# kakaoenterprise/JORLDY

Measured on AMD Instinct MI355X. Metric: env_steps_per_s (PPO CartPole sync, W=8 workers/GPU, T=128), higher is better.
Workload: dtype f32

## Files before the change

jorldy_amd/csrc/jh_collect.hip:

```cpp
#include <chrono>

#include "jh_common.h"

struct jh_persist;
int jh_persist_create(jh_pponet* n, jh_persist** out);
void jh_persist_destroy(jh_persist* p);
int jh_persist_begin(jh_persist* p, int W, int T, hipStream_t st, int split = 0);
unsigned jh_persist_publish(jh_persist* p, int W, const float* h_obs);
unsigned jh_persist_seq(const jh_persist* p);
void jh_persist_publish_rows(jh_persist* p, int r0, int r1, const float* h_obs, unsigned tag);
int jh_persist_collect_range(jh_persist* p, int r0, int n_rows, unsigned tag, float* h_heads);
int jh_persist_collect(jh_persist* p, int W, unsigned tag, float* h_heads);
int jh_persist_collect_rows(jh_persist* p, const int* rows, int n_rows, unsigned tag, float* h_heads);
void jh_persist_abort(jh_persist* p);
bool jh_persist_gave_up(const jh_persist* p);
void jh_persist_dump_debug(jh_persist* p, int T);

namespace {
struct Level {
  void* env = nullptr;
  int S = 0;
  std::vector<float> next, obs, rw;
  std::vector<uint8_t> dn;
  std::vector<int64_t> act;
  void init(int rows, int S_) {
    S = S_;
    next.resize((size_t)S * rows); obs.resize((size_t)S * rows); rw.resize(rows); dn.resize(rows); act.resize(rows);
    for (int i = 0; i < rows; ++i) act[i] = i & 1;
  }
};
inline int fork_step(const jh_env_vtbl& vt, Level& dst, const void* src, int n_src) {
  for (int i = 0; i < n_src; ++i) { vt.copy_row(dst.env, 2 * i, src, i); vt.copy_row(dst.env, 2 * i + 1, src, i); }
  int rc = vt.step(dst.env, 0, 2 * n_src, dst.act.data(), dst.next.data(), dst.rw.data(), dst.dn.data());
  if (rc) return rc;
  return vt.obs(dst.env, 0, 2 * n_src, dst.obs.data());
}
inline void copy_level_row(const jh_env_vtbl& vt, Level& d, int di, const Level& s_, int si) {
  vt.copy_row(d.env, di, s_.env, si);
  const size_t S = (size_t)d.S;
  memcpy(&d.next[S * (size_t)di], &s_.next[S * (size_t)si], sizeof(float) * S);
  memcpy(&d.obs[S * (size_t)di], &s_.obs[S * (size_t)si], sizeof(float) * S);
  d.rw[di] = s_.rw[si];
  d.dn[di] = s_.dn[si];
}
}

struct jh_collector {
  jh_ctx* ctx = nullptr;
  jh_pponet* net = nullptr;
  jh_env_vtbl vt{};
// ... 1 lines not shown
  jh_store* store = nullptr;
  int W = 0, S = 0, A = 0;
  int no = 0;
  bool cont = false;
  int col_state = 0, col_action = 1, col_reward = 2, col_next = 3, col_done = 4;
  std::vector<float> obs, next_obs, reward, heads, act_f;
  std::vector<int64_t> act_i;
  std::vector<uint8_t> done;
  bool dbg = false, dbg_persist = false;
  double dbg_publish = 0.0, dbg_wait = 0.0;
  long dbg_n = 0;
  jh_persist* persist = nullptr;
  int mode = 1;
  int lookahead = 1;
  bool split = false;
  Level lv[4];
  void *spec = nullptr, *spec2 = nullptr, *spec3 = nullptr;
  float *cap_h0 = nullptr, *cap_h1 = nullptr, *cap_v = nullptr, *cap_nv = nullptr;
  int64_t cap_rows = 0;
  const void* ride_src[2] = {nullptr, nullptr};
  void* ride_dst[2] = {nullptr, nullptr};
  int64_t ride_bytes[2] = {0, 0};
  void* run = nullptr;
  unsigned *gate_h = nullptr, *gate_d = nullptr, gate_seq = 0;
  int prelaunched_T = 0;
  double t_act = 0, t_env = 0, t_total = 0;
  double t_first = 0, t_extra = 0, t_commit = 0;
  int64_t runs = 0;
  int64_t steps = 0;
};
// ... 28 lines not shown
  c->dbg = getenv("JH_COLLECT_DEBUG") != nullptr;
  c->dbg_persist = getenv("JH_PERSIST_DEBUG") != nullptr;
  if (const char* e = getenv("JH_COLLECT_PERSISTENT")) c->mode = atoi(e);
  if (c->mode == 1 && W <= 32 && W * S <= 512) {
    if (jh_persist_create(net, &c->persist) != JH_OK) c->persist = nullptr;
  }
  const bool forkable = vt->fork_alloc && vt->fork_free && vt->copy_row;
  if (c->persist && forkable && !cont && A == 2 && 3 * W <= 32 && 3 * W * S <= 128) {
    const char* e = getenv("JH_COLLECT_LOOKAHEAD");
    c->lookahead = e ? (atoi(e) >= 2 ? 2 : 1) : 2;
    if (c->lookahead == 2) {
      c->spec = vt->fork_alloc(env, 2 * W); c->spec2 = vt->fork_alloc(env, 4 * W); c->spec3 = vt->fork_alloc(env, 8 * W);
      if (!c->spec || !c->spec2 || !c->spec3) c->lookahead = 1;
    }
  }
  {
    const char* e = getenv("JH_COLLECT_SPLIT");
    c->split = c->persist && c->lookahead != 2 && W == 32 && (vt->obs == cart_obs || vt->obs == ctl_obs) && !(e && atoi(e) == 0);
  }
  c->obs.resize((size_t)S * W);
  c->next_obs.resize((size_t)S * W);
  c->act_i.resize(W);
  c->act_f.resize((size_t)A * W);
  c->reward.resize(W);
  c->done.resize(W);
  c->heads.resize((size_t)c->no * W);
  run_state_alloc(c);
  *out = c;
  return JH_OK;
}

static int cart_obs(void* e, int32_t r0, int32_t r1, float* o) { jh_cartpole_obs_rows((const jh_cartpole*)e, r0, r1, o); return JH_OK; }
static int cart_step(void* e, int32_t r0, int32_t r1, const void* a, float* nx, float* rw, uint8_t* dn) {
// ... 72 lines not shown
  JH_ARG(c != nullptr && slot >= 0 && slot < 2 && bytes >= 0 && (bytes == 0 || (d_src_mapped && d_dst)));
  c->ride_src[slot] = d_src_mapped; c->ride_dst[slot] = d_dst; c->ride_bytes[slot] = bytes;
  return JH_OK;
}

static int collector_steps(const jh_collector* c, int T) {
  const int extra = (c->cap_v && c->cap_rows == (int64_t)c->W * T) ? 1 : 0;
  return (c->lookahead == 2 ? (T + 1) / 2 : T) + extra;
}
static int collector_rows(const jh_collector* c) { return c->lookahead == 2 ? 3 * c->W : c->W; }

JH_EXPORT int jh_collector_prelaunch(jh_collector* c, int32_t T, jh_stream stream) {
  JH_ARG(c != nullptr && T > 0);
  if (!c->persist || c->prelaunched_T) return JH_OK;
  const int steps = collector_steps(c, T);
  int rc = jh_persist_begin(c->persist, collector_rows(c), steps, jh_s(stream), c->split);
  if (rc == JH_OK) c->prelaunched_T = steps;
  return rc;
}

struct RunState {
  bool active = false, cap = false, persistent = false, early = false;
  int T = 0, steps = 0;
  int64_t n = 0;
  float *st = nullptr, *ns = nullptr, *rw = nullptr;
  uint8_t* dn = nullptr;
  int64_t* ac_i = nullptr;
  float* ac_f = nullptr;
  jh_pinned_slab* cap_slab = nullptr;
  float *ch0 = nullptr, *ch1 = nullptr, *cv = nullptr, *cnv = nullptr;
  int stall_t = -1, stall_h = -1;
// ... 63 lines not shown
    if (rc) { (void)jh_store_stage_commit(c->store, st); return rc; }
    r.ch0 = (float*)r.cap_slab->host;
    r.ch1 = c->cont ? r.ch0 + (size_t)r.n * A : nullptr;
    r.cv = r.ch0 + (size_t)r.n * A * (c->cont ? 2 : 1);
    r.cnv = r.cv + r.n;
  }
  r.persistent = c->persist != nullptr;
  if (r.persistent) {
    const int pre = c->prelaunched_T;
    c->prelaunched_T = 0;
    if (pre != r.steps || jh_persist_gave_up(c->persist)) {
      if (pre && !jh_persist_gave_up(c->persist)) {
        jh_persist_abort(c->persist);
        (void)hipStreamSynchronize(st);
      }
      rc = jh_persist_begin(c->persist, collector_rows(c), r.steps, st, c->split);
      if (rc) r.persistent = false;
    }
  }
  r.active = true;
  return JH_OK;
}

using Clock = std::chrono::steady_clock;
static double secs(Clock::time_point a, Clock::time_point b) { return std::chrono::duration<double>(b - a).count(); }

static void count_act(jh_collector* c, const RunState& r, int t, double dt) {
  c->t_act += dt;
  if (t == r.T) c->t_extra += dt;
  else if (t == 0) c->t_first += dt;
}
// ... 102 lines not shown
    c->steps += 1;
  }
  *t_done = steps;
  if (c->dbg_persist && (c->runs % 16) == 15) jh_persist_dump_debug(c->persist, T);
  if (c->dbg_n > 0 && (c->runs % 4) == 3) {
    fprintf(stderr, "[jh_collect] one timestep per exchange, per step: publish %.2f us, wait + read of the heads %.2f us (sampling + bookkeeping + env step: the rest of act / env)\n",
            c->dbg_publish / c->dbg_n * 1e6, c->dbg_wait / c->dbg_n * 1e6);
    c->dbg_publish = c->dbg_wait = 0.0;
    c->dbg_n = 0;
  }
  return JH_OK;
}

static int run_loop_split(jh_collector* c, int training, hipStream_t st, int* t_done) {
  RunState& r = run_state(c);
  const int W = c->W, T = r.T, steps = T + (r.cap ? 1 : 0), HR = 16;
  const unsigned base = jh_persist_seq(c->persist);
  bool dead = false;
  int rc = c->vt.obs(c->env, 0, W, c->obs.data());
  if (rc) return env_failed(c, rc);
  for (int h = 0; h < 2; ++h) jh_persist_publish_rows(c->persist, h * HR, (h + 1) * HR, c->obs.data(), base + 1);
  for (int t = 0; t < steps; ++t) {
    const bool extra = t == T;
    for (int h = 0; h < 2; ++h) {
      const int r0 = h * HR, r1 = r0 + HR;
      const auto t0 = Clock::now();
      if (t == r.stall_t && h == r.stall_h) {
        while (secs(t0, Clock::now()) < 0.35) {}
      }
      rc = jh_persist_collect_range(c->persist, r0, HR, base + (unsigned)t + 1, c->heads.data() + (size_t)r0 * c->no);
      if (rc) {
        rc = kernel_gave_up(c, r, t, st, t_done);
        if (rc || h == 0) return rc;
        const uint64_t ctr = c->net->act_ctr;
        rc = act_launch(c, r0, HR, 0, st);
        if (rc) return rc;
        c->net->act_ctr = ctr;
        dead = true;
      }
      for (int w = r0; w < r1; ++w) {
        const float* z = c->heads.data() + (size_t)w * c->no;
        if (!extra) sample_row(c, z, w, training);
        capture_row(c, r, w, t, z);
      }
      if (h == 1 && !extra) c->net->act_ctr += 1;
      const auto t1 = Clock::now();
      count_act(c, r, t, secs(t0, t1));
      if (extra) continue;
      rc = step_rows(c, r, r0, r1, t);
      if (rc) return env_failed(c, rc);
      if (t + 1 < steps && !dead) {
        rc = c->vt.obs(c->env, r0, r1, c->obs.data());
        if (rc) return env_failed(c, rc);
        jh_persist_publish_rows(c->persist, r0, r1, c->obs.data(), base + (unsigned)t + 2);
      }
      c->t_env += secs(t1, Clock::now());
    }
    if (!extra) c->steps += 1;
    if (dead) {
      *t_done = t + 1;
      return JH_OK;
    }
  }
  *t_done = steps;
  return JH_OK;
}

static int run_loop_lookahead(jh_collector* c, int training, hipStream_t st, int* t_done) {
  RunState& r = run_state(c);
  const int W = c->W, S = c->S, T = r.T, steps = T + (r.cap ? 1 : 0), no = c->no;
  void* e = c->env;
  const jh_env_vtbl& vt = c->vt;
  Level &L1 = c->lv[0], &L2 = c->lv[1], &L3 = c->lv[2], &tmp = c->lv[3];
  L1.env = c->spec; L2.env = c->spec2; L3.env = c->spec3;
  L1.init(2 * W, S); L2.init(4 * W, S); L3.init(8 * W, S);
  std::vector<float> pub((size_t)3 * W * S), pub_next((size_t)3 * W * S), hz((size_t)W * no), hz2((size_t)W * no);
  std::vector<int> pick(W);
  std::vector<int64_t> a0(W), a1(W);
  int t = 0;
  const bool dbg = c->dbg;
  double d_fork = 0, d_wait = 0, d_sample = 0, d_publish = 0, d_book = 0;
  int n_ex = 0;
  int rc = fork_step(vt, L1, e, W);
  if (!rc) rc = vt.obs(e, 0, W, pub.data());
  if (rc) return env_failed(c, rc);
  memcpy(pub.data() + (size_t)W * S, L1.obs.data(), sizeof(float) * (size_t)2 * W * S);
  auto t0 = Clock::now();
  unsigned tag = jh_persist_publish(c->persist, 3 * W, pub.data());
  while (t < steps) {
    const bool extra = t == T;
    const bool two = !extra && t + 1 < T;
    const int t_next = t + (two ? 2 : 1);
    const auto q0 = dbg ? Clock::now() : Clock::time_point();
    if (!extra) {
      rc = fork_step(vt, L2, L1.env, 2 * W);
      if (!rc && two && t_next < steps) rc = fork_step(vt, L3, L2.env, 4 * W);
      if (rc) return env_failed(c, rc);
    }
    const auto q1 = dbg ? Clock::now() : q0;
    rc = jh_persist_collect_rows(c->persist, nullptr, W, tag, hz.data());
    const auto q2 = dbg ? Clock::now() : q0;
    if (rc) return kernel_gave_up(c, r, t, st, t_done);
    if (!extra) {
      for (int w = 0; w < W; ++w) {
        a0[w] = jh_sample_discrete(c->net, hz.data() + (size_t)w * no, w, training);
        pick[w] = W + 2 * w + (int)a0[w];
      }
      c->net->act_ctr += 1;
      if (two) {
        rc = jh_persist_collect_rows(c->persist, pick.data(), W, tag, hz2.data());
        if (rc) return rc;
// ... 52 lines not shown
    if (!two)
      for (int i = 0; i < 2 * W; ++i) copy_level_row(vt, L1, i, tmp, i);
    c->steps += two ? 2 : 1;
    const auto t2 = Clock::now();
    if (dbg) d_book += secs(q3, t2);
    c->t_env += secs(t1, t2);
    t = t_next;
    tag = tag_next;
    t0 = t0_next;
    pub.swap(pub_next);
  }
  *t_done = t;
  if (dbg && n_ex > 0 && (c->runs % 16) == 15)
    fprintf(stderr, "[jh_collect] host us per exchange (%d exchanges): fork %.2f  wait %.2f  sample %.2f  publish %.2f  book %.2f\n", n_ex, d_fork / n_ex * 1e6,
            d_wait / n_ex * 1e6, d_sample / n_ex * 1e6, d_publish / n_ex * 1e6, d_book / n_ex * 1e6);
  if (c->dbg_persist && (c->runs % 16) == 15) jh_persist_dump_debug(c->persist, collector_steps(c, T));
  return JH_OK;
}

static int run_loop_per_launch(jh_collector* c, int training, hipStream_t st, int t_begin) {
  RunState& r = run_state(c);
  if (r.early) return jh_fail(JH_ERR_STATE, "jh_collector_begin needs the persistent acting kernel (W <= 32, W * S <= 512, JH_COLLECT_PERSISTENT != 0)");
  const int W = c->W, T = r.T, steps = T + (r.cap ? 1 : 0);
  for (int t = t_begin; t < steps; ++t) {
    const bool extra = t == T;
    int rc = c->vt.obs(c->env, 0, W, c->obs.data());
    if (rc) return rc;
    const auto t0 = Clock::now();
    rc = act_launch(c, 0, W, training, st);
    if (rc) return rc;
// ... 2 lines not shown
    const auto t1 = Clock::now();
    count_act(c, r, t, secs(t0, t1));
    if (extra) break;
    rc = step_rows(c, r, 0, W, t);
    if (rc) return rc;
    c->t_env += secs(t1, Clock::now());
    c->steps += 1;
  }
  return JH_OK;
}

static int run_loop(jh_collector* c, int training, hipStream_t st) {
  RunState& r = run_state(c);
  int t = 0;
  if (r.persistent) {
    const int rc = c->lookahead == 2 ? run_loop_lookahead(c, training, st, &t)
                   : c->split        ? run_loop_split(c, training, st, &t)
                                     : run_loop_exchange(c, training, st, &t);
    if (rc) return rc;
  }
  return t < r.T + (r.cap ? 1 : 0) ? run_loop_per_launch(c, training, st, t) : JH_OK;
}

JH_EXPORT int jh_collector_run(jh_collector* c, int32_t T, int32_t training, jh_stream stream) {
  JH_ARG(c != nullptr && T > 0);
  if (run_state(c).active) return jh_fail(JH_ERR_STATE, "jh_collector_run inside a jh_collector_begin / jh_collector_loop pair");
  int rc = run_prepare(c, T, jh_s(stream));
  if (rc) return rc;
  rc = run_loop(c, training, jh_s(stream));
  const auto tc = std::chrono::steady_clock::now();
  rc = run_commit(c, run_state(c), rc, nullptr, 0, jh_s(stream));
// ... 75 lines not shown
```

jorldy_amd/csrc/jh_common.h:

```cpp
#pragma once
#include <hip/hip_runtime.h>
#include <math.h>
#include <stdint.h>
#include <stdio.h>
#include <string.h>

#include <deque>
#include <mutex>
#include <string>
#include <vector>

#include "../../include/jorldy_hip.h"

#define JH_EXPORT extern "C" __attribute__((visibility("default")))

std::string& jh_err_slot();
int jh_fail(int code, const char* fmt, ...);

#define JH_HIP(expr)                                                                          \
  do {                                                                                        \
    hipError_t _e = (expr);                                                                   \
    if (_e != hipSuccess)                                                                     \
      return jh_fail(JH_ERR_HIP, "%s:%d %s -> %s", __FILE__, __LINE__, #expr, hipGetErrorString(_e)); \
  } while (0)
// ... 143 lines not shown
  float* xg = nullptr;
  float* tg_ws = nullptr;
  size_t tg_ws_floats = 0;
  unsigned* tg_cnt = nullptr;
  int tg_cnt_slots = 0;
};

static inline uint64_t jh_mix64(uint64_t x) {
  x += 0x9E3779B97F4A7C15ull;
  x = (x ^ (x >> 30)) * 0xBF58476D1CE4E5B9ull;
  x = (x ^ (x >> 27)) * 0x94D049BB133111EBull;
  return x ^ (x >> 31);
}
static inline double jh_u01_of(uint64_t key) { return (double)(jh_mix64(key) >> 11) * (1.0 / 9007199254740992.0); }

static inline int64_t jh_sample_discrete(const jh_pponet* n, const float* z, int wq, int training) {
  const int A = n->A;
  int act = 0;
  float mx = z[0];
  for (int k = 1; k < A; ++k)
    if (z[k] > mx) { mx = z[k]; act = k; }
  if (!training) return act;
  float e[40], se = 0.f;
  for (int k = 0; k < A; ++k) { e[k] = expf(z[k] - mx); se += e[k]; }
  const float u = (float)jh_u01_of(n->act_seed * 0x100000001B3ull + n->act_ctr * 0x9E3779B97F4A7C15ull + (uint64_t)wq) * se;
  float c = 0.f;
  act = A - 1;
  for (int k = 0; k < A; ++k) {
    c += e[k];
    if (u < c) { act = k; break; }
  }
  return act;
}

static inline void jh_sample_continuous(const jh_pponet* n, const float* z, int wq, int training, float* action) {
  const int A = n->A;
  for (int k = 0; k < A; ++k) {
    const float mu = fminf(fmaxf(z[k], -5.f), 5.f);
    float v = mu;
    if (training) {
      const float sd = expf(tanhf(z[A + k]));
      const uint64_t key = n->act_seed * 0x100000001B3ull + n->act_ctr * 0x9E3779B97F4A7C15ull + (uint64_t)wq * 64u + (uint64_t)k;
      const double u1 = 1.0 - jh_u01_of(key * 2 + 1), u2 = jh_u01_of(key * 2 + 2);
      v = mu + sd * (float)(sqrt(-2.0 * log(u1)) * cos(6.283185307179586 * u2));
    }
    action[k] = tanhf(v);
  }
}
// ... 75 lines not shown
```

jorldy_amd/csrc/jh_persist.hip:

```cpp
#if defined(__x86_64__)
#include <emmintrin.h>
#endif

#include "jh_common.h"

typedef float f32x4 __attribute__((ext_vector_type(4)));

struct PersistArgs {
  int W, S, H, n_out, T, G;
  const float *W1, *b1, *W2, *b2;
  const float* wh[12];
  const float* hbias[12];
  const unsigned long long* obs_gran;
  float4* part;
  int rows_ld;
  unsigned* abort_flag;
  unsigned seq0;
  long max_polls;
  unsigned long long* dbg;
  int period;
  unsigned long long* mbox;
  float4* dpart;
  int split;
};

__device__ __forceinline__ void persist_poll_issue(const void* gsrc, unsigned lds_off) {
  unsigned keep;
  asm volatile("s_mov_b32 %0, m0\n\ts_mov_b32 m0, %2\n\ts_nop 0\n\tglobal_load_lds_dwordx4 %1, off sc0 sc1\n\ts_mov_b32 m0, %0"
               : "=&s"(keep) : "v"(gsrc), "s"(lds_off) : "memory");
}

template <int SP, int NCH, int D, int PI>
__global__ void __launch_bounds__(256, 1) jh_act_persist_kernel(PersistArgs p) {
  constexpr bool W1LDS = SP > 8;
  constexpr int NJ = 2 * PI;
  __shared__ __attribute__((aligned(16))) unsigned long long s_ring[D][128 * PI];
  __shared__ __attribute__((aligned(16))) float s_w1[W1LDS ? 64 * NCH * SP : 4];
  __shared__ __attribute__((aligned(16))) float s_x[2][16][SP];
// ... 29 lines not shown
      const int k = i / SP, q = i - k * SP;
      s_w1[i] = q < S ? p.W1[(size_t)k * S + q] : 0.f;
    }
  }
  for (int i = threadIdx.x; i < 12 * 16; i += 256) {
    const int o = i >> 4, c = i & 15;
    s_wh[o][c] = o < p.n_out ? p.wh[o][n0 + c] : 0.f;
  }
  if (threadIdx.x < 16) s_b2[threadIdx.x] = p.b2[n0 + threadIdx.x];
  if (threadIdx.x < 12) s_hb[threadIdx.x] = threadIdx.x < p.n_out ? *p.hbias[threadIdx.x] : 0.f;
  for (int i = threadIdx.x; i < 2 * 16 * SP; i += 256) (&s_x[0][0][0])[i] = 0.f;
  for (int i = threadIdx.x; i < D * 128 * PI; i += 256) (&s_ring[0][0])[i] = 0ull;
  __syncthreads();

  const int g0 = p.split ? rt * 16 * S : 0;
  const int n_gran = p.split ? (p.W - 16 * rt < 16 ? p.W - 16 * rt : 16) * S : p.W * S;
  const int n16 = (n_gran + 1) >> 1;
  const char* my_src = reinterpret_cast<const char*>(p.obs_gran + g0) + 16 * (lane < n16 ? lane : 0);
  const bool poller = !p.mbox || (p.split ? tile == 0 : blockIdx.x == 0);
  unsigned long long next_issue = 0;
  int slot = 0;
  const unsigned ring_lane = (unsigned)(uintptr_t)&s_ring[0][0] + 8u * (unsigned)lane;
  __builtin_amdgcn_s_waitcnt(0x0F70);
  if (wid == 0 && poller) {
#pragma unroll
    for (int d = 0; d < D; ++d) {
#pragma unroll
      for (int q = 0; q < PI; ++q)
        if (64 * q + lane < n16) persist_poll_issue(my_src + 1024 * q, __builtin_amdgcn_readfirstlane((unsigned)(uintptr_t)&s_ring[d][0]) + 1024u * q);
    }
    next_issue = wall_clock64();
// ... 127 lines not shown
      __builtin_amdgcn_fence(__ATOMIC_RELEASE, "workgroup");
      f32x4 ph = (f32x4){0.f, 0.f, 0.f, 0.f};
#pragma unroll
      for (int c = 0; c < 4; ++c) {
        const float av = s_h2[r][4 * c + kq];
        const float bv = r < 12 ? s_wh[r][4 * c + kq] : 0.f;
        ph = __builtin_amdgcn_mfma_f32_16x16x4f32(av, bv, ph, 0, 0, 0);
      }
      if (r < 12) {
#pragma unroll
        for (int i = 0; i < 4; ++i) s_out[kq * 4 + i][r] = ph[i] + (tile == 0 ? s_hb[r] : 0.f);
      }
      __builtin_amdgcn_wave_barrier();
      __builtin_amdgcn_fence(__ATOMIC_RELEASE, "workgroup");
      const int g = lane >> 4, row = lane & 15;
      if (g < p.G && 16 * rt + row < p.W) {
        const f32x4 gq = (f32x4){s_out[row][3 * g], s_out[row][3 * g + 1], s_out[row][3 * g + 2], __uint_as_float(tag)};
        if (p.dpart) {
          float4* dst = p.dpart + ((size_t)(rt * p.G + g) * 16 + row) * tiles_n + tile;
          asm volatile("global_store_dwordx4 %0, %1, off sc1\n\ts_nop 1" ::"v"(dst), "v"(gq) : "memory");
        } else {
          float4* dst = p.part + ((size_t)tile * p.G + g) * p.rows_ld + 16 * rt + row;
          asm volatile("global_store_dwordx4 %0, %1, off sc0 sc1\n\ts_nop 1" ::"v"(dst), "v"(gq) : "memory");
        }
      }
    }
    if (p.dpart && tile == 0) {
      const int g = lane >> 4, row = lane & 15;
      const bool mine = g < p.G && 16 * rt + row < p.W;
      const int per = tiles_n / 4;
      bool ok = true;
      if (mine) {
        const float4* src = p.dpart + ((size_t)(rt * p.G + g) * 16 + row) * tiles_n + wid * per;
        f32x4 q[8];
        long spin = 0;
        for (;;) {
          const float4* a1 = per > 4 ? src + 4 : src;
          asm volatile("global_load_dwordx4 %0, %8, off sc1\n\tglobal_load_dwordx4 %1, %9, off sc1\n\tglobal_load_dwordx4 %2, %10, off sc1\n\t"
                       "global_load_dwordx4 %3, %11, off sc1\n\tglobal_load_dwordx4 %4, %12, off sc1\n\tglobal_load_dwordx4 %5, %12, off offset:16 sc1\n\t"
                       "global_load_dwordx4 %6, %12, off offset:32 sc1\n\tglobal_load_dwordx4 %7, %12, off offset:48 sc1\n\ts_waitcnt vmcnt(0)"
                       : "=&v"(q[0]), "=&v"(q[1]), "=&v"(q[2]), "=&v"(q[3]), "=&v"(q[4]), "=&v"(q[5]), "=&v"(q[6]), "=&v"(q[7])
                       : "v"(src), "v"(src + (per > 1 ? 1 : 0)), "v"(src + (per > 2 ? 2 : 0)), "v"(src + (per > 2 ? 3 : 0)), "v"(a1)
                       : "memory");
          bool all = true, newer = false;
// ... 21 lines not shown
          good = good && __float_as_uint(v[3]) == tag;
          z0 += v[0]; z1 += v[1]; z2 += v[2];
        }
        if (good) {
          const f32x4 gq = (f32x4){z0, z1, z2, __uint_as_float(tag)};
          float4* dst = p.part + (size_t)g * p.rows_ld + 16 * rt + row;
          asm volatile("global_store_dwordx4 %0, %1, off sc0 sc1\n\ts_nop 1" ::"v"(dst), "v"(gq) : "memory");
        }
      }
    }
    if (p.dbg && blockIdx.x == 0 && threadIdx.x == 0) { p.dbg[(t - 1) * 8 + 4] = wall_clock64(); p.dbg[(t - 1) * 8 + 5] = __builtin_readcyclecounter(); }
  }
  asm volatile("s_waitcnt vmcnt(0)" ::: "memory");
}

constexpr int kPersistMaxGranules = 512;
struct jh_persist {
  jh_pponet* net = nullptr;
  unsigned long long* gran_h = nullptr;
  unsigned long long* gran_d = nullptr;
  float4 *part_h = nullptr, *part_d = nullptr;
  unsigned *flag_h = nullptr, *flag_d = nullptr;
  unsigned seq = 0;
  int tiles = 0, n_out = 0, G = 0;
  int rows_ld = 16;
  unsigned long long *dbg_h = nullptr, *dbg_d = nullptr;
  unsigned long long* mbox = nullptr;
  float4* dpart = nullptr;
  bool reduced = false;
  int rows_published = 0;
// ... 40 lines not shown
  (void)hipHostFree(p->part_h);
  (void)hipHostFree(p->flag_h);
  (void)hipFree(p->mbox);
  (void)hipFree(p->dpart);
  if (p->dbg_d) (void)hipFree(p->dbg_d);
  free(p->dbg_h);
  delete p;
}

template <int SP, int NCH>
static void persist_launch(int depth, int pi, int grid, hipStream_t st, const PersistArgs& a) {
  if (pi == 2) JH_LAUNCH_NAMED("jh_act_persist_kernel", (jh_act_persist_kernel<SP, NCH, 4, 2>), dim3(grid), dim3(256), 0, st, a);
  else if (pi == 3) JH_LAUNCH_NAMED("jh_act_persist_kernel", (jh_act_persist_kernel<SP, NCH, 4, 3>), dim3(grid), dim3(256), 0, st, a);
  else if (pi == 4) JH_LAUNCH_NAMED("jh_act_persist_kernel", (jh_act_persist_kernel<SP, NCH, 4, 4>), dim3(grid), dim3(256), 0, st, a);
  else if (depth >= 4) JH_LAUNCH_NAMED("jh_act_persist_kernel", (jh_act_persist_kernel<SP, NCH, 4, 1>), dim3(grid), dim3(256), 0, st, a);
  else if (depth >= 2) JH_LAUNCH_NAMED("jh_act_persist_kernel", (jh_act_persist_kernel<SP, NCH, 2, 1>), dim3(grid), dim3(256), 0, st, a);
  else JH_LAUNCH_NAMED("jh_act_persist_kernel", (jh_act_persist_kernel<SP, NCH, 1, 1>), dim3(grid), dim3(256), 0, st, a);
}

int jh_persist_begin(jh_persist* p, int W, int T, hipStream_t st, int split) {
  jh_pponet* n = p->net;
  JH_ARG(W > 0 && W <= 32 && W * n->S <= kPersistMaxGranules && T > 0 && (!split || W == 32));
  const int win = split ? 16 * n->S : W * n->S;
  const int pi = ((win + 1) / 2 + 63) / 64;
  PersistArgs a{};
  a.W = W; a.S = n->S; a.H = n->H; a.T = T; a.G = p->G;
  a.W1 = n->params + n->o_w1; a.b1 = n->params + n->o_b1; a.W2 = n->params + n->o_w2; a.b2 = n->params + n->o_b2;
  int o = 0;
  for (int k = 0; k < n->A; ++k, ++o) { a.wh[o] = n->params + n->o_wh0 + (int64_t)k * n->H; a.hbias[o] = n->params + n->o_bh0 + k; }
  if (n->cont)
    for (int k = 0; k < n->A; ++k, ++o) { a.wh[o] = n->params + n->o_wh1 + (int64_t)k * n->H; a.hbias[o] = n->params + n->o_bh1 + k; }
  a.wh[o] = n->params + n->o_wv; a.hbias[o] = n->params + n->o_bv; ++o;
  a.n_out = o;
  a.obs_gran = p->gran_d; a.part = p->part_d; a.abort_flag = p->flag_d;
  a.seq0 = p->seq;
  a.dbg = p->dbg_d;
  static const int depth = getenv("JH_PERSIST_DEPTH") ? atoi(getenv("JH_PERSIST_DEPTH")) : 4;
  static const int period = getenv("JH_PERSIST_PERIOD") ? atoi(getenv("JH_PERSIST_PERIOD")) : 10;
  a.period = depth > 1 ? period : 0;
  static const int relay = getenv("JH_PERSIST_RELAY") ? atoi(getenv("JH_PERSIST_RELAY")) : 1;
  a.mbox = relay ? p->mbox : nullptr;
  const int reduce = getenv("JH_PERSIST_REDUCE") ? atoi(getenv("JH_PERSIST_REDUCE")) : (split ? 1 : 0);
  p->reduced = reduce == 1;
  a.dpart = p->reduced ? p->dpart : nullptr;
  a.split = split ? 1 : 0;
  p->split = split != 0;
  a.max_polls = 600000;
  p->flag_h[0] = 0;
  const int nch = n->H / 64;
  const int sp = (n->S + 3) / 4 * 4;
  const int rt = W > 16 ? 2 : 1;
  p->rows_ld = 16 * rt;
  a.rows_ld = p->rows_ld;
  const int grid = p->tiles * rt;
#define JH_PERSIST_CASE(NCH)                                   \
  if (nch == NCH) {                                            \
    if (sp == 4) persist_launch<4, NCH>(depth, pi, grid, st, a);   \
    else if (sp == 8) persist_launch<8, NCH>(depth, pi, grid, st, a);   \
    else if (sp == 12) persist_launch<12, NCH>(depth, pi, grid, st, a); \
    else persist_launch<16, NCH>(depth, pi, grid, st, a);          \
  }
  JH_PERSIST_CASE(1) else JH_PERSIST_CASE(2) else JH_PERSIST_CASE(4) else JH_PERSIST_CASE(8)
#undef JH_PERSIST_CASE
  JH_LAUNCH_CHECK();
  return JH_OK;
}

unsigned jh_persist_publish(jh_persist* p, int W, const float* h_obs) {
  const unsigned tag = ++p->seq;
  p->rows_published = W;
  const int n = W * p->net->S;
  for (int i = 0; i < n; ++i) {
    unsigned bits;
    memcpy(&bits, h_obs + i, 4);
    __atomic_store_n(p->gran_h + i, ((unsigned long long)tag << 32) | bits, __ATOMIC_RELEASE);
  }
  return tag;
}

unsigned jh_persist_seq(const jh_persist* p) { return p->seq; }
void jh_persist_publish_rows(jh_persist* p, int r0, int r1, const float* h_obs, unsigned tag) {
  const int S = p->net->S;
  if (r1 > p->rows_published) p->rows_published = r1;
  for (int i = r0 * S; i < r1 * S; ++i) {
    unsigned bits;
    memcpy(&bits, h_obs + i, 4);
    __atomic_store_n(p->gran_h + i, ((unsigned long long)tag << 32) | bits, __ATOMIC_RELEASE);
  }
  if ((int)(tag - p->seq) > 0) p->seq = tag;
}

static int persist_collect(jh_persist* p, const int* rows, int n_rows, unsigned tag, float* h_heads, int r_first, bool block_order);
int jh_persist_collect_rows(jh_persist* p, const int* rows, int n_rows, unsigned tag, float* h_heads) {
  return persist_collect(p, rows, n_rows, tag, h_heads, 0, !rows && n_rows > 16);
}
int jh_persist_collect_range(jh_persist* p, int r0, int n_rows, unsigned tag, float* h_heads) { return persist_collect(p, nullptr, n_rows, tag, h_heads, r0, true); }
static int persist_collect(jh_persist* p, const int* rows, int n_rows, unsigned tag, float* h_heads, int r_first, bool block_order) {
  const int n_out = p->n_out, G = p->G, ld = p->rows_ld, tiles = p->reduced ? 1 : p->tiles;
  volatile unsigned* abort_w = p->flag_h;
  struct alignas(16) Gran16 { unsigned w[4]; };
  const Gran16* part = reinterpret_cast<const Gran16*>(p->part_h);
  float z[32][12];
  unsigned char have[32];
  JH_ARG(n_rows <= 32);
  if (block_order) {
    for (int k = 0; k < n_rows; ++k)
      for (int o = 0; o < 12; ++o) z[k][o] = 0.f;
    long spins = 0;
    for (int t = 0; t < tiles; ++t)
      for (int g = 0; g < G; ++g) {
        const Gran16* blk = part + ((size_t)t * G + g) * ld + r_first;
        for (;;) {
// ... 10 lines not shown
#if defined(__x86_64__)
          _mm_store_si128(reinterpret_cast<__m128i*>(w4), _mm_load_si128(reinterpret_cast<const __m128i*>(blk + k)));
#else
          memcpy(w4, blk + k, 16);
#endif
          if (w4[3] != tag) return jh_fail(JH_ERR_STATE, "persistent acting kernel: granule of step tag %u rewritten while it was read", tag);
          float f3[3];
          memcpy(f3, w4, 12);
          z[k][3 * g] += f3[0]; z[k][3 * g + 1] += f3[1]; z[k][3 * g + 2] += f3[2];
        }
      }
    for (int k = 0; k < n_rows; ++k) memcpy(h_heads + (size_t)k * n_out, z[k], sizeof(float) * n_out);
    return JH_OK;
  }
  int missing = n_rows;
  const int pf_rows = (!rows && p->rows_published > n_rows) ? p->rows_published - n_rows : 0;
  for (int k = 0; k < n_rows; ++k) have[k] = 0;
  for (long spin = 0; spin < 40000000L && missing; ++spin) {
    for (int k = 0; k < n_rows; ++k) {
      if (have[k]) continue;
      const int wq = rows ? rows[k] : k;
      float acc[12] = {0, 0, 0, 0, 0, 0, 0, 0, 0, 0, 0, 0};
      bool ok = true;
      for (int t = 0; t < tiles && ok; ++t)
        for (int g = 0; g < G; ++g) {
          const Gran16* gp = part + ((size_t)t * G + g) * ld + wq;
          if (__atomic_load_n(reinterpret_cast<const unsigned*>(gp) + 3, __ATOMIC_ACQUIRE) != tag) { ok = false; break; }
#if defined(__x86_64__)
          if (pf_rows > 0 && k == 0) {
            const char* q = reinterpret_cast<const char*>(part + ((size_t)t * G + g) * ld + n_rows);
            for (int b = 0; b < pf_rows * 16; b += 64) _mm_prefetch(q + b, _MM_HINT_T0);
          }
#endif
          alignas(16) unsigned w4[4];
#if defined(__x86_64__)
          _mm_store_si128(reinterpret_cast<__m128i*>(w4), _mm_load_si128(reinterpret_cast<const __m128i*>(gp)));
#else
          memcpy(w4, gp, 16);
#endif
          if (w4[3] != tag) { ok = false; break; }
          float f3[3];
          memcpy(f3, w4, 12);
          acc[3 * g] += f3[0]; acc[3 * g + 1] += f3[1]; acc[3 * g + 2] += f3[2];
        }
      if (ok) {
// ... 40 lines not shown
```

Before: 1.119 million.

## Split lookahead collection into two env halves pipelined against persistent kernel

```diff
diff --git a/jorldy_amd/csrc/jh_collect.hip b/jorldy_amd/csrc/jh_collect.hip
--- a/jorldy_amd/csrc/jh_collect.hip
+++ b/jorldy_amd/csrc/jh_collect.hip
@@ -5,11 +5,13 @@
 struct jh_persist;
 int jh_persist_create(jh_pponet* n, jh_persist** out);
 void jh_persist_destroy(jh_persist* p);
-int jh_persist_begin(jh_persist* p, int W, int T, hipStream_t st, int split = 0);
+bool jh_persist_can_split(const jh_persist* p, int rows_a, int rows_b);
+int jh_persist_begin(jh_persist* p, int W, int T, hipStream_t st, const int* half_rows = nullptr);
 unsigned jh_persist_publish(jh_persist* p, int W, const float* h_obs);
 unsigned jh_persist_seq(const jh_persist* p);
-void jh_persist_publish_rows(jh_persist* p, int r0, int r1, const float* h_obs, unsigned tag);
+void jh_persist_publish_at(jh_persist* p, int row0, int n_rows, const float* h_obs, unsigned tag);
 int jh_persist_collect_range(jh_persist* p, int r0, int n_rows, unsigned tag, float* h_heads);
+int jh_persist_collect_half(jh_persist* p, int r_first, const int* rows, int n_rows, int pf_rows, unsigned tag, float* h_heads);
 int jh_persist_collect(jh_persist* p, int W, unsigned tag, float* h_heads);
 int jh_persist_collect_rows(jh_persist* p, const int* rows, int n_rows, unsigned tag, float* h_heads);
 void jh_persist_abort(jh_persist* p);
@@ -29,11 +31,11 @@
     for (int i = 0; i < rows; ++i) act[i] = i & 1;
   }
 };
-inline int fork_step(const jh_env_vtbl& vt, Level& dst, const void* src, int n_src) {
-  for (int i = 0; i < n_src; ++i) { vt.copy_row(dst.env, 2 * i, src, i); vt.copy_row(dst.env, 2 * i + 1, src, i); }
-  int rc = vt.step(dst.env, 0, 2 * n_src, dst.act.data(), dst.next.data(), dst.rw.data(), dst.dn.data());
+inline int fork_step(const jh_env_vtbl& vt, Level& dst, const void* src, int i0, int i1) {
+  for (int i = i0; i < i1; ++i) { vt.copy_row(dst.env, 2 * i, src, i); vt.copy_row(dst.env, 2 * i + 1, src, i); }
+  int rc = vt.step(dst.env, 2 * i0, 2 * i1, dst.act.data(), dst.next.data(), dst.rw.data(), dst.dn.data());
   if (rc) return rc;
-  return vt.obs(dst.env, 0, 2 * n_src, dst.obs.data());
+  return vt.obs(dst.env, 2 * i0, 2 * i1, dst.obs.data());
 }
 inline void copy_level_row(const jh_env_vtbl& vt, Level& d, int di, const Level& s_, int si) {
   vt.copy_row(d.env, di, s_.env, si);
@@ -65,6 +67,7 @@
   int mode = 1;
   int lookahead = 1;
   bool split = false;
+  int half_envs[2] = {0, 0}, half_rows[2] = {0, 0};
   Level lv[4];
   void *spec = nullptr, *spec2 = nullptr, *spec3 = nullptr;
   float *cap_h0 = nullptr, *cap_h1 = nullptr, *cap_v = nullptr, *cap_nv = nullptr;
@@ -123,9 +126,14 @@
       if (!c->spec || !c->spec2 || !c->spec3) c->lookahead = 1;
     }
   }
-  {
+  if (c->persist && W >= 2) {
     const char* e = getenv("JH_COLLECT_SPLIT");
-    c->split = c->persist && c->lookahead != 2 && W == 32 && (vt->obs == cart_obs || vt->obs == ctl_obs) && !(e && atoi(e) == 0);
+    const int per_env = c->lookahead == 2 ? 3 : 1;
+    c->half_envs[0] = (W + 1) / 2; c->half_envs[1] = W - c->half_envs[0];
+    for (int h = 0; h < 2; ++h) c->half_rows[h] = per_env * c->half_envs[h];
+    const bool can = (c->lookahead == 2 ? vt->obs == cart_obs : (vt->obs == cart_obs || vt->obs == ctl_obs)) &&
+                     jh_persist_can_split(c->persist, c->half_rows[0], c->half_rows[1]);
+    c->split = can && !(e && atoi(e) == 0);
   }
   c->obs.resize((size_t)S * W);
   c->next_obs.resize((size_t)S * W);
@@ -228,7 +236,7 @@
   JH_ARG(c != nullptr && T > 0);
   if (!c->persist || c->prelaunched_T) return JH_OK;
   const int steps = collector_steps(c, T);
-  int rc = jh_persist_begin(c->persist, collector_rows(c), steps, jh_s(stream), c->split);
+  int rc = jh_persist_begin(c->persist, collector_rows(c), steps, jh_s(stream), c->split ? c->half_rows : nullptr);
   if (rc == JH_OK) c->prelaunched_T = steps;
   return rc;
 }
@@ -322,7 +330,7 @@
         jh_persist_abort(c->persist);
         (void)hipStreamSynchronize(st);
       }
-      rc = jh_persist_begin(c->persist, collector_rows(c), r.steps, st, c->split);
+      rc = jh_persist_begin(c->persist, collector_rows(c), r.steps, st, c->split ? c->half_rows : nullptr);
       if (rc) r.persistent = false;
     }
   }
@@ -455,26 +463,26 @@
 
 static int run_loop_split(jh_collector* c, int training, hipStream_t st, int* t_done) {
   RunState& r = run_state(c);
-  const int W = c->W, T = r.T, steps = T + (r.cap ? 1 : 0), HR = 16;
+  const int W = c->W, S = c->S, T = r.T, steps = T + (r.cap ? 1 : 0);
   const unsigned base = jh_persist_seq(c->persist);
   bool dead = false;
   int rc = c->vt.obs(c->env, 0, W, c->obs.data());
   if (rc) return env_failed(c, rc);
-  for (int h = 0; h < 2; ++h) jh_persist_publish_rows(c->persist, h * HR, (h + 1) * HR, c->obs.data(), base + 1);
+  for (int h = 0; h < 2; ++h) jh_persist_publish_at(c->persist, 16 * h, c->half_envs[h], c->obs.data() + (size_t)S * (h ? c->half_envs[0] : 0), base + 1);
   for (int t = 0; t < steps; ++t) {
     const bool extra = t == T;
     for (int h = 0; h < 2; ++h) {
-      const int r0 = h * HR, r1 = r0 + HR;
+      const int r0 = h ? c->half_envs[0] : 0, r1 = r0 + c->half_envs[h];
       const auto t0 = Clock::now();
       if (t == r.stall_t && h == r.stall_h) {
         while (secs(t0, Clock::now()) < 0.35) {}
       }
-      rc = jh_persist_collect_range(c->persist, r0, HR, base + (unsigned)t + 1, c->heads.data() + (size_t)r0 * c->no);
+      rc = jh_persist_collect_range(c->persist, 16 * h, r1 - r0, base + (unsigned)t + 1, c->heads.data() + (size_t)r0 * c->no);
       if (rc) {
         rc = kernel_gave_up(c, r, t, st, t_done);
         if (rc || h == 0) return rc;
         const uint64_t ctr = c->net->act_ctr;
-        rc = act_launch(c, r0, HR, 0, st);
+        rc = act_launch(c, r0, r1 - r0, 0, st);
         if (rc) return rc;
         c->net->act_ctr = ctr;
         dead = true;
@@ -493,7 +501,7 @@
       if (t + 1 < steps && !dead) {
         rc = c->vt.obs(c->env, r0, r1, c->obs.data());
         if (rc) return env_failed(c, rc);
-        jh_persist_publish_rows(c->persist, r0, r1, c->obs.data(), base + (unsigned)t + 2);
+        jh_persist_publish_at(c->persist, 16 * h, r1 - r0, c->obs.data() + (size_t)S * r0, base + (unsigned)t + 2);
       }
       c->t_env += secs(t1, Clock::now());
     }
@@ -522,7 +530,7 @@
   const bool dbg = c->dbg;
   double d_fork = 0, d_wait = 0, d_sample = 0, d_publish = 0, d_book = 0;
   int n_ex = 0;
-  int rc = fork_step(vt, L1, e, W);
+  int rc = fork_step(vt, L1, e, 0, W);
   if (!rc) rc = vt.obs(e, 0, W, pub.data());
   if (rc) return env_failed(c, rc);
   memcpy(pub.data() + (size_t)W * S, L1.obs.data(), sizeof(float) * (size_t)2 * W * S);
@@ -533,9 +541,12 @@
     const bool two = !extra && t + 1 < T;
     const int t_next = t + (two ? 2 : 1);
     const auto q0 = dbg ? Clock::now() : Clock::time_point();
+    if (t == r.stall_t && r.stall_h == 0) {
+      while (secs(t0, Clock::now()) < 0.35) {}
+    }
     if (!extra) {
-      rc = fork_step(vt, L2, L1.env, 2 * W);
-      if (!rc && two && t_next < steps) rc = fork_step(vt, L3, L2.env, 4 * W);
+      rc = fork_step(vt, L2, L1.env, 0, 2 * W);
+      if (!rc && two && t_next < steps) rc = fork_step(vt, L3, L2.env, 0, 4 * W);
       if (rc) return env_failed(c, rc);
     }
     const auto q1 = dbg ? Clock::now() : q0;
@@ -618,6 +629,180 @@
   if (dbg && n_ex > 0 && (c->runs % 16) == 15)
     fprintf(stderr, "[jh_collect] host us per exchange (%d exchanges): fork %.2f  wait %.2f  sample %.2f  publish %.2f  book %.2f\n", n_ex, d_fork / n_ex * 1e6,
             d_wait / n_ex * 1e6, d_sample / n_ex * 1e6, d_publish / n_ex * 1e6, d_book / n_ex * 1e6);
+  if (c->dbg_persist && (c->runs % 16) == 15) jh_persist_dump_debug(c->persist, collector_steps(c, T));
+  return JH_OK;
+}
+
+namespace {
+struct LookHalf {
+  int e0 = 0, e1 = 0, row0 = 0;
+  int t = 0;
+  unsigned tag = 0;
+  std::vector<float> pub, pub_next, hz, hz2;
+  std::vector<int> pick;
+  std::vector<int64_t> a0, a1;
+  double d_fork = 0, d_wait = 0, d_sample = 0, d_publish = 0, d_book = 0;
+  int n_ex = 0;
+};
+}
+
+static int run_loop_lookahead_halves(jh_collector* c, int training, hipStream_t st, int* t_done) {
+  RunState& r = run_state(c);
+  const int W = c->W, S = c->S, T = r.T, steps = T + (r.cap ? 1 : 0), no = c->no;
+  void* e = c->env;
+  const jh_env_vtbl& vt = c->vt;
+  Level &L1 = c->lv[0], &L2 = c->lv[1], &L3 = c->lv[2], &tmp = c->lv[3];
+  L1.env = c->spec; L2.env = c->spec2; L3.env = c->spec3;
+  L1.init(2 * W, S); L2.init(4 * W, S); L3.init(8 * W, S);
+  tmp.env = L3.env; tmp.init(2 * W, S);
+  const bool dbg = c->dbg;
+  const uint64_t ctr0 = c->net->act_ctr;
+  const unsigned base = jh_persist_seq(c->persist);
+  bool dead = false;
+  LookHalf hf[2];
+  for (int h = 0; h < 2; ++h) {
+    LookHalf& H = hf[h];
+    H.e0 = h ? c->half_envs[0] : 0; H.e1 = H.e0 + c->half_envs[h]; H.row0 = 16 * h;
+    const int E = H.e1 - H.e0;
+    H.pub.resize((size_t)3 * E * S); H.pub_next.resize((size_t)3 * E * S); H.hz.resize((size_t)E * no); H.hz2.resize((size_t)E * no);
+    H.pick.resize(E); H.a0.resize(E); H.a1.resize(E);
+  }
+  auto fork_ahead = [&](LookHalf& H) -> int {
+    if (H.t >= T) return JH_OK;
+    const bool two = H.t + 1 < T;
+    int rc = fork_step(vt, L2, L1.env, 2 * H.e0, 2 * H.e1);
+    if (!rc && two && H.t + 2 < steps) rc = fork_step(vt, L3, L2.env, 4 * H.e0, 4 * H.e1);
+    return rc;
+  };
+  auto heads_of = [&](LookHalf& H, bool chosen, float* out) -> int {
+    const int E = H.e1 - H.e0;
+    if (dead && !chosen) {
+      const int rc = jh_persist_begin(c->persist, 3 * E, 1, st);
+      if (rc) return rc;
+      H.row0 = 0;
+      H.tag = jh_persist_publish(c->persist, 3 * E, H.pub.data());
+    }
+    return jh_persist_collect_half(c->persist, H.row0, chosen ? H.pick.data() : nullptr, E, chosen ? 0 : 2 * E, H.tag, out);
+  };
+  int rc = vt.obs(e, 0, W, c->obs.data());
+  if (rc) return env_failed(c, rc);
+  auto prev_end = Clock::now();
+  for (int h = 0; h < 2; ++h) {
+    LookHalf& H = hf[h];
+    const int E = H.e1 - H.e0;
+    rc = fork_step(vt, L1, e, H.e0, H.e1);
+    if (rc) return env_failed(c, rc);
+    memcpy(H.pub.data(), &c->obs[(size_t)S * H.e0], sizeof(float) * (size_t)E * S);
+    memcpy(H.pub.data() + (size_t)E * S, &L1.obs[(size_t)S * 2 * H.e0], sizeof(float) * (size_t)2 * E * S);
+    H.tag = base + 1;
+    if (h == 0) prev_end = Clock::now();
+    jh_persist_publish_at(c->persist, H.row0, 3 * E, H.pub.data(), H.tag);
+    rc = fork_ahead(H);
+    if (rc) return env_failed(c, rc);
+  }
+  for (int x = 0; x < r.steps; ++x) {
+    for (int h = 0; h < 2; ++h) {
+      LookHalf& H = hf[h];
+      const int E = H.e1 - H.e0, t = H.t;
+      const bool extra = t == T;
+      const bool two = !extra && t + 1 < T;
+      const int t_next = t + (two ? 2 : 1);
+      const auto s0 = prev_end;
+      if (t == r.stall_t && h == r.stall_h) {
+        const auto z0 = Clock::now();
+        while (secs(z0, Clock::now()) < 0.35) {}
+      }
+      const auto q1 = dbg ? Clock::now() : s0;
+      rc = heads_of(H, false, H.hz.data());
+      if (rc && !dead) {
+        c->net->act_ctr = ctr0 + (uint64_t)(hf[0].t < T ? hf[0].t : T);
+        rc = kernel_gave_up(c, r, hf[0].t, st, t_done);
+        if (rc || h == 0) return rc;
+        dead = true;
+        rc = heads_of(H, false, H.hz.data());
+      }
+      if (rc) return rc;
+      const auto q2 = dbg ? Clock::now() : s0;
+      if (!extra) {
+        for (int k = 0; k < E; ++k) {
+          H.a0[k] = jh_sample_discrete_at(c->net, H.hz.data() + (size_t)k * no, H.e0 + k, training, ctr0 + (uint64_t)t);
+          H.pick[k] = E + 2 * k + (int)H.a0[k];
+        }
+        if (two) {
+          rc = heads_of(H, true, H.hz2.data());
+          if (rc) return rc;
+          for (int k = 0; k < E; ++k) H.a1[k] = jh_sample_discrete_at(c->net, H.hz2.data() + (size_t)k * no, H.e0 + k, training, ctr0 + (uint64_t)t + 1);
+        }
+      }
+      const auto t1 = Clock::now();
+      double dt_pub = 0.0;
+      if (!extra && t_next < steps && !dead) {
+        for (int k = 0; k < E; ++k) {
+          const int k1 = 2 * (H.e0 + k) + (int)H.a0[k];
+          if (two) {
+            const int k2 = 2 * k1 + (int)H.a1[k];
+            memcpy(&H.pub_next[(size_t)S * k], &L2.obs[(size_t)S * k2], sizeof(float) * S);
+            memcpy(&H.pub_next[(size_t)S * (E + 2 * k)], &L3.obs[(size_t)S * 2 * k2], sizeof(float) * 2 * S);
+          } else {
+            memcpy(&H.pub_next[(size_t)S * k], &L1.obs[(size_t)S * k1], sizeof(float) * S);
+            memcpy(&H.pub_next[(size_t)S * (E + 2 * k)], &L2.obs[(size_t)S * 2 * k1], sizeof(float) * 2 * S);
+          }
+        }
+        const auto p0 = Clock::now();
+        jh_persist_publish_at(c->persist, H.row0, 3 * E, H.pub_next.data(), H.tag + 1);
+        dt_pub = secs(p0, Clock::now());
+      }
+      const auto q3 = dbg ? Clock::now() : t1;
+      for (int k = 0; k < E; ++k) {
+        capture_row(c, r, H.e0 + k, t, H.hz.data() + (size_t)k * no);
+        if (two) capture_row(c, r, H.e0 + k, t + 1, H.hz2.data() + (size_t)k * no);
+      }
+      if (!extra) {
+        for (int k = 0; k < E; ++k) {
+          const int w = H.e0 + k, k1 = 2 * w + (int)H.a0[k];
+          store_row(c, r, w, t, &H.pub[(size_t)S * k], &L1.next[(size_t)S * k1], &H.a0[k], L1.rw[k1], L1.dn[k1]);
+          if (two) {
+            const int k2 = 2 * k1 + (int)H.a1[k];
+            store_row(c, r, w, t + 1, &L1.obs[(size_t)S * k1], &L2.next[(size_t)S * k2], &H.a1[k], L2.rw[k2], L2.dn[k2]);
+            vt.copy_row(e, w, L2.env, k2);
+            if (t_next < steps) {
+              copy_level_row(vt, L1, 2 * w, L3, 2 * k2);
+              copy_level_row(vt, L1, 2 * w + 1, L3, 2 * k2 + 1);
+            }
+          } else {
+            vt.copy_row(e, w, L1.env, k1);
+            copy_level_row(vt, tmp, 2 * w, L2, 2 * k1);
+            copy_level_row(vt, tmp, 2 * w + 1, L2, 2 * k1 + 1);
+          }
+        }
+        if (!two)
+          for (int i = 2 * H.e0; i < 2 * H.e1; ++i) copy_level_row(vt, L1, i, tmp, i);
+        if (h == 1) c->steps += two ? 2 : 1;
+      }
+      const auto t2 = Clock::now();
+      H.t = t_next;
+      H.tag += 1;
+      H.pub.swap(H.pub_next);
+      if (!dead) {
+        rc = fork_ahead(H);
+        if (rc) return env_failed(c, rc);
+      }
+      const auto t3 = Clock::now();
+      count_act(c, r, t, secs(s0, t1) + dt_pub + secs(t2, t3));
+      c->t_env += secs(t1, t2);
+      if (dbg) { H.d_wait += secs(q1, q2); H.d_sample += secs(q2, t1); H.d_publish += secs(t1, q3); H.d_book += secs(q3, t2); H.d_fork += secs(t2, t3); ++H.n_ex; }
+      prev_end = t3;
+    }
+    if (dead) break;
+  }
+  *t_done = hf[1].t;
+  c->net->act_ctr = ctr0 + (uint64_t)(hf[1].t < T ? hf[1].t : T);
+  if (dbg && hf[0].n_ex > 0 && (c->runs % 16) == 15)
+    for (int h = 0; h < 2; ++h) {
+      const LookHalf& H = hf[h];
+      fprintf(stderr, "[jh_collect] half %d (%d envs), host us per exchange (%d exchanges): fork %.2f  wait %.2f  sample %.2f  publish %.2f  book %.2f\n", h, H.e1 - H.e0,
+              H.n_ex, H.d_fork / H.n_ex * 1e6, H.d_wait / H.n_ex * 1e6, H.d_sample / H.n_ex * 1e6, H.d_publish / H.n_ex * 1e6, H.d_book / H.n_ex * 1e6);
+    }
   if (c->dbg_persist && (c->runs % 16) == 15) jh_persist_dump_debug(c->persist, collector_steps(c, T));
   return JH_OK;
 }
@@ -650,7 +835,7 @@
   RunState& r = run_state(c);
   int t = 0;
   if (r.persistent) {
-    const int rc = c->lookahead == 2 ? run_loop_lookahead(c, training, st, &t)
+    const int rc = c->lookahead == 2 ? (c->split ? run_loop_lookahead_halves(c, training, st, &t) : run_loop_lookahead(c, training, st, &t))
                    : c->split        ? run_loop_split(c, training, st, &t)
                                      : run_loop_exchange(c, training, st, &t);
     if (rc) return rc;
diff --git a/jorldy_amd/csrc/jh_common.h b/jorldy_amd/csrc/jh_common.h
--- a/jorldy_amd/csrc/jh_common.h
+++ b/jorldy_amd/csrc/jh_common.h
@@ -181,7 +181,7 @@
 }
 static inline double jh_u01_of(uint64_t key) { return (double)(jh_mix64(key) >> 11) * (1.0 / 9007199254740992.0); }
 
-static inline int64_t jh_sample_discrete(const jh_pponet* n, const float* z, int wq, int training) {
+static inline int64_t jh_sample_discrete_at(const jh_pponet* n, const float* z, int wq, int training, uint64_t ctr) {
   const int A = n->A;
   int act = 0;
   float mx = z[0];
@@ -190,7 +190,7 @@
   if (!training) return act;
   float e[40], se = 0.f;
   for (int k = 0; k < A; ++k) { e[k] = expf(z[k] - mx); se += e[k]; }
-  const float u = (float)jh_u01_of(n->act_seed * 0x100000001B3ull + n->act_ctr * 0x9E3779B97F4A7C15ull + (uint64_t)wq) * se;
+  const float u = (float)jh_u01_of(n->act_seed * 0x100000001B3ull + ctr * 0x9E3779B97F4A7C15ull + (uint64_t)wq) * se;
   float c = 0.f;
   act = A - 1;
   for (int k = 0; k < A; ++k) {
@@ -199,6 +199,7 @@
   }
   return act;
 }
+static inline int64_t jh_sample_discrete(const jh_pponet* n, const float* z, int wq, int training) { return jh_sample_discrete_at(n, z, wq, training, n->act_ctr); }
 
 static inline void jh_sample_continuous(const jh_pponet* n, const float* z, int wq, int training, float* action) {
   const int A = n->A;
diff --git a/jorldy_amd/csrc/jh_persist.hip b/jorldy_amd/csrc/jh_persist.hip
--- a/jorldy_amd/csrc/jh_persist.hip
+++ b/jorldy_amd/csrc/jh_persist.hip
@@ -22,6 +22,7 @@
   unsigned long long* mbox;
   float4* dpart;
   int split;
+  int half_rows[2];
 };
 
 __device__ __forceinline__ void persist_poll_issue(const void* gsrc, unsigned lds_off) {
@@ -81,7 +82,8 @@
   __syncthreads();
 
   const int g0 = p.split ? rt * 16 * S : 0;
-  const int n_gran = p.split ? (p.W - 16 * rt < 16 ? p.W - 16 * rt : 16) * S : p.W * S;
+  const int my_rows = p.split ? (rt ? p.half_rows[1] : p.half_rows[0]) : (p.W - 16 * rt < 16 ? p.W - 16 * rt : 16);
+  const int n_gran = p.split ? my_rows * S : p.W * S;
   const int n16 = (n_gran + 1) >> 1;
   const char* my_src = reinterpret_cast<const char*>(p.obs_gran + g0) + 16 * (lane < n16 ? lane : 0);
   const bool poller = !p.mbox || (p.split ? tile == 0 : blockIdx.x == 0);
@@ -239,7 +241,7 @@
       __builtin_amdgcn_wave_barrier();
       __builtin_amdgcn_fence(__ATOMIC_RELEASE, "workgroup");
       const int g = lane >> 4, row = lane & 15;
-      if (g < p.G && 16 * rt + row < p.W) {
+      if (g < p.G && row < my_rows) {
         const f32x4 gq = (f32x4){s_out[row][3 * g], s_out[row][3 * g + 1], s_out[row][3 * g + 2], __uint_as_float(tag)};
         if (p.dpart) {
           float4* dst = p.dpart + ((size_t)(rt * p.G + g) * 16 + row) * tiles_n + tile;
@@ -252,7 +254,7 @@
     }
     if (p.dpart && tile == 0) {
       const int g = lane >> 4, row = lane & 15;
-      const bool mine = g < p.G && 16 * rt + row < p.W;
+      const bool mine = g < p.G && row < my_rows;
       const int per = tiles_n / 4;
       bool ok = true;
       if (mine) {
@@ -304,6 +306,7 @@
   asm volatile("s_waitcnt vmcnt(0)" ::: "memory");
 }
 
+constexpr int kPersistSplitDepth = 4;
 constexpr int kPersistMaxGranules = 512;
 struct jh_persist {
   jh_pponet* net = nullptr;
@@ -374,15 +377,26 @@
   else if (pi == 3) JH_LAUNCH_NAMED("jh_act_persist_kernel", (jh_act_persist_kernel<SP, NCH, 4, 3>), dim3(grid), dim3(256), 0, st, a);
   else if (pi == 4) JH_LAUNCH_NAMED("jh_act_persist_kernel", (jh_act_persist_kernel<SP, NCH, 4, 4>), dim3(grid), dim3(256), 0, st, a);
   else if (depth >= 4) JH_LAUNCH_NAMED("jh_act_persist_kernel", (jh_act_persist_kernel<SP, NCH, 4, 1>), dim3(grid), dim3(256), 0, st, a);
+  else if (depth == 3) JH_LAUNCH_NAMED("jh_act_persist_kernel", (jh_act_persist_kernel<SP, NCH, 3, 1>), dim3(grid), dim3(256), 0, st, a);
   else if (depth >= 2) JH_LAUNCH_NAMED("jh_act_persist_kernel", (jh_act_persist_kernel<SP, NCH, 2, 1>), dim3(grid), dim3(256), 0, st, a);
   else JH_LAUNCH_NAMED("jh_act_persist_kernel", (jh_act_persist_kernel<SP, NCH, 1, 1>), dim3(grid), dim3(256), 0, st, a);
 }
 
-int jh_persist_begin(jh_persist* p, int W, int T, hipStream_t st, int split) {
+static int persist_poll_instructions(int granules) { return ((granules + 1) / 2 + 63) / 64; }
+
+bool jh_persist_can_split(const jh_persist* p, int rows_a, int rows_b) {
+  const int S = p->net->S;
+  return rows_a >= 1 && rows_a <= 16 && rows_b >= 1 && rows_b <= 16 && persist_poll_instructions(rows_a * S) == persist_poll_instructions(rows_b * S);
+}
+
+int jh_persist_begin(jh_persist* p, int W, int T, hipStream_t st, const int* half_rows) {
   jh_pponet* n = p->net;
-  JH_ARG(W > 0 && W <= 32 && W * n->S <= kPersistMaxGranules && T > 0 && (!split || W == 32));
-  const int win = split ? 16 * n->S : W * n->S;
-  const int pi = ((win + 1) / 2 + 63) / 64;
+  const bool split = half_rows != nullptr;
+  JH_ARG(W > 0 && W <= 32 && W * n->S <= kPersistMaxGranules && T > 0);
+  JH_ARG(!split || (jh_persist_can_split(p, half_rows[0], half_rows[1]) && W == half_rows[0] + half_rows[1]));
+  const bool full = split && W == 32;
+  const int win = split ? half_rows[0] * n->S : W * n->S;
+  const int pi = persist_poll_instructions(win);
   PersistArgs a{};
   a.W = W; a.S = n->S; a.H = n->H; a.T = T; a.G = p->G;
   a.W1 = n->params + n->o_w1; a.b1 = n->params + n->o_b1; a.W2 = n->params + n->o_w2; a.b2 = n->params + n->o_b2;
@@ -395,21 +409,24 @@
   a.obs_gran = p->gran_d; a.part = p->part_d; a.abort_flag = p->flag_d;
   a.seq0 = p->seq;
   a.dbg = p->dbg_d;
-  static const int depth = getenv("JH_PERSIST_DEPTH") ? atoi(getenv("JH_PERSIST_DEPTH")) : 4;
+  static const int depth_env = getenv("JH_PERSIST_DEPTH") ? atoi(getenv("JH_PERSIST_DEPTH")) : 0;
+  const int depth = depth_env > 0 ? depth_env : (split && !full ? kPersistSplitDepth : 4);
   static const int period = getenv("JH_PERSIST_PERIOD") ? atoi(getenv("JH_PERSIST_PERIOD")) : 10;
   a.period = depth > 1 ? period : 0;
   static const int relay = getenv("JH_PERSIST_RELAY") ? atoi(getenv("JH_PERSIST_RELAY")) : 1;
   a.mbox = relay ? p->mbox : nullptr;
-  const int reduce = getenv("JH_PERSIST_REDUCE") ? atoi(getenv("JH_PERSIST_REDUCE")) : (split ? 1 : 0);
+  const int reduce = getenv("JH_PERSIST_REDUCE") ? atoi(getenv("JH_PERSIST_REDUCE")) : (full ? 1 : 0);
   p->reduced = reduce == 1;
   a.dpart = p->reduced ? p->dpart : nullptr;
   a.split = split ? 1 : 0;
-  p->split = split != 0;
+  a.half_rows[0] = split ? half_rows[0] : 0;
+  a.half_rows[1] = split ? half_rows[1] : 0;
+  p->split = split;
   a.max_polls = 600000;
   p->flag_h[0] = 0;
   const int nch = n->H / 64;
   const int sp = (n->S + 3) / 4 * 4;
-  const int rt = W > 16 ? 2 : 1;
+  const int rt = (split || W > 16) ? 2 : 1;
   p->rows_ld = 16 * rt;
   a.rows_ld = p->rows_ld;
   const int grid = p->tiles * rt;
@@ -439,23 +456,27 @@
 }
 
 unsigned jh_persist_seq(const jh_persist* p) { return p->seq; }
-void jh_persist_publish_rows(jh_persist* p, int r0, int r1, const float* h_obs, unsigned tag) {
+void jh_persist_publish_at(jh_persist* p, int row0, int n_rows, const float* h_obs, unsigned tag) {
   const int S = p->net->S;
-  if (r1 > p->rows_published) p->rows_published = r1;
-  for (int i = r0 * S; i < r1 * S; ++i) {
+  unsigned long long* g = p->gran_h + (size_t)row0 * S;
+  for (int i = 0; i < n_rows * S; ++i) {
     unsigned bits;
     memcpy(&bits, h_obs + i, 4);
-    __atomic_store_n(p->gran_h + i, ((unsigned long long)tag << 32) | bits, __ATOMIC_RELEASE);
+    __atomic_store_n(g + i, ((unsigned long long)tag << 32) | bits, __ATOMIC_RELEASE);
   }
   if ((int)(tag - p->seq) > 0) p->seq = tag;
 }
 
-static int persist_collect(jh_persist* p, const int* rows, int n_rows, unsigned tag, float* h_heads, int r_first, bool block_order);
+static int persist_collect(jh_persist* p, const int* rows, int n_rows, unsigned tag, float* h_heads, int r_first, bool block_order, int pf_rows);
 int jh_persist_collect_rows(jh_persist* p, const int* rows, int n_rows, unsigned tag, float* h_heads) {
-  return persist_collect(p, rows, n_rows, tag, h_heads, 0, !rows && n_rows > 16);
-}
-int jh_persist_collect_range(jh_persist* p, int r0, int n_rows, unsigned tag, float* h_heads) { return persist_collect(p, nullptr, n_rows, tag, h_heads, r0, true); }
-static int persist_collect(jh_persist* p, const int* rows, int n_rows, unsigned tag, float* h_heads, int r_first, bool block_order) {
+  const int pf_rows = (!rows && p->rows_published > n_rows) ? p->rows_published - n_rows : 0;
+  return persist_collect(p, rows, n_rows, tag, h_heads, 0, !rows && n_rows > 16, pf_rows);
+}
+int jh_persist_collect_half(jh_persist* p, int r_first, const int* rows, int n_rows, int pf_rows, unsigned tag, float* h_heads) {
+  return persist_collect(p, rows, n_rows, tag, h_heads, r_first, false, rows ? 0 : pf_rows);
+}
+int jh_persist_collect_range(jh_persist* p, int r0, int n_rows, unsigned tag, float* h_heads) { return persist_collect(p, nullptr, n_rows, tag, h_heads, r0, true, 0); }
+static int persist_collect(jh_persist* p, const int* rows, int n_rows, unsigned tag, float* h_heads, int r_first, bool block_order, int pf_rows) {
   const int n_out = p->n_out, G = p->G, ld = p->rows_ld, tiles = p->reduced ? 1 : p->tiles;
   volatile unsigned* abort_w = p->flag_h;
   struct alignas(16) Gran16 { unsigned w[4]; };
@@ -496,12 +517,11 @@
     return JH_OK;
   }
   int missing = n_rows;
-  const int pf_rows = (!rows && p->rows_published > n_rows) ? p->rows_published - n_rows : 0;
   for (int k = 0; k < n_rows; ++k) have[k] = 0;
   for (long spin = 0; spin < 40000000L && missing; ++spin) {
     for (int k = 0; k < n_rows; ++k) {
       if (have[k]) continue;
-      const int wq = rows ? rows[k] : k;
+      const int wq = r_first + (rows ? rows[k] : k);
       float acc[12] = {0, 0, 0, 0, 0, 0, 0, 0, 0, 0, 0, 0};
       bool ok = true;
       for (int t = 0; t < tiles && ok; ++t)
@@ -510,7 +530,7 @@
           if (__atomic_load_n(reinterpret_cast<const unsigned*>(gp) + 3, __ATOMIC_ACQUIRE) != tag) { ok = false; break; }
 #if defined(__x86_64__)
           if (pf_rows > 0 && k == 0) {
-            const char* q = reinterpret_cast<const char*>(part + ((size_t)t * G + g) * ld + n_rows);
+            const char* q = reinterpret_cast<const char*>(part + ((size_t)t * G + g) * ld + r_first + n_rows);
             for (int b = 0; b < pf_rows * 16; b += 64) _mm_prefetch(q + b, _MM_HINT_T0);
           }
 #endif
```

Result: slower. 972,000 (-13.1%).
